# CAS-CLab/quantized-cnn

Measured on AMD Instinct MI355X. Metric: images/sec AlexNet quantized forward, higher is better.
Workload: dtype f32

## Files before the change

### quantized-cnn_amd/csrc/qcnn_decoded.hip

```cpp
#include "qcnn_kernels.h"
#include <algorithm>
#include <type_traits>

typedef float f32x4 __attribute__((ext_vector_type(4)));

#ifndef QCNN_DEC_VAR
#define QCNN_DEC_VAR 0
#endif

namespace {

constexpr int PANEL = QCNN_PANEL;

__device__ __forceinline__ int uni(int v) { return __builtin_amdgcn_readfirstlane(v); }

__host__ __device__ __forceinline__ int qk_dec_krow(int k, int Kr, int Kp) {
  const int last = Kp - 4;
  if (k < last || Kr < 4) return k < Kr ? k : -1;
  const int real = Kr - 4 + (k - last);
  return real >= last ? real : -1;
}

__global__ void k_decode_weights(const uint8_t* __restrict__ rows, const float* __restrict__ ctrd, float* __restrict__ out,
                                 QkSlots sl, int knl, int Cin, int K, int Ct, int Kp, int S) {
  const int total = knl * Kp * S;
  for (int i = blockIdx.x * blockDim.x + threadIdx.x; i < total; i += gridDim.x * blockDim.x) {
    const int ch = i % S, k = qk_dec_krow((i / S) % Kp, knl * Cin, Kp), kh = i / (S * Kp);
    float w = 0.0f;
    if (ch < Ct && k >= 0) {
      const int kw = k / Cin, d = k % Cin;
      const int slot = rows[(size_t)(kh * knl + kw) * sl.rowStride + qk_slot_entry(sl, 0, ch)];
      w = ctrd[(size_t)d * K + qcnn_row_slot(slot)];
    }
    out[i] = w;
  }
}

template <int CT, int PW, bool PADDED, int R, int IT>
__global__ __launch_bounds__(1024) void k_conv_dec(DecParams p) {
  extern __shared__ __attribute__((aligned(16))) float ldsW[];
  const int lane = threadIdx.x & 63, wave = uni(threadIdx.x >> 6);
  const int P = p.Ho * p.Wo;
  {
    const int wq = (p.knl * p.Kp * p.S) >> 2;
    const f32x4* __restrict__ wsrc = reinterpret_cast<const f32x4*>(p.wdec);
    f32x4* ldsW4 = reinterpret_cast<f32x4*>(ldsW);
    for (int i = threadIdx.x; i < wq; i += 1024) ldsW4[i] = wsrc[i];
  }
  __syncthreads();
  const int NS = p.Kp >> 2;
  const int T = p.knl * NS;
  const int groups = (P + PW - 1) / PW;
  constexpr int IB = 16 * IT;
  const int halves = (p.live + IB - 1) / IB;
  const int chunks = p.Ct / (16 * CT);
  const int nItems = p.panels * groups * halves * chunks;
  const int kClamp = p.Kr - 1;
  const int xcd = blockIdx.x & 7, nX = gridDim.x < 8 ? gridDim.x : 8;
  const int wgX = (gridDim.x - xcd + 7) >> 3;
  const int itemBeg = (int)((long long)nItems * xcd / nX), itemEnd = (int)((long long)nItems * (xcd + 1) / nX);
  for (int item = itemBeg + (blockIdx.x >> 3) * 16 + wave; item < itemEnd; item += wgX * 16) {
    int laneI = lane;
    asm volatile("" : "+v"(laneI));
    const int li = laneI & 15, kq = laneI >> 4;
    const int cc = item % chunks, ib = (item / chunks) % halves, pgi = item / (chunks * halves);
    const int panel = pgi / groups, pos0 = (pgi % groups) * PW;
    int r0[PW], c0[PW];
#pragma unroll
    for (int j = 0; j < PW; ++j) {
      const int q = pos0 + j < P ? pos0 + j : P - 1;
      r0[j] = (q / p.Wo) * p.stride - p.pad;
      c0[j] = (q % p.Wo) * p.stride - p.pad;
    }
    const float* __restrict__ srcU = p.src + (size_t)panel * p.H * p.W * p.Cin * PANEL + ib * IB;
    const size_t left = (size_t)(p.panels - panel) * p.H * p.W * p.Cin * PANEL * sizeof(float) - ib * IB * sizeof(float);
    const __amdgpu_buffer_rsrc_t rsrc = __builtin_amdgcn_make_buffer_rsrc(
        const_cast<float*>(srcU), 0, left < 0xffffffffull ? (unsigned)left : 0xffffffffu, 0x00020000);
    const int laneOff = (kq * PANEL + IT * li) * (int)sizeof(float);
    int posOff[PW];
#pragma unroll
    for (int j = 0; j < PW; ++j) posOff[j] = (r0[j] * p.W + c0[j]) * p.Cin * PANEL * (int)sizeof(float);
    const int rowPitch = p.W * p.Cin * PANEL * (int)sizeof(float);
    constexpr int kStep = 4 * PANEL * (int)sizeof(float);
    auto load_b = [&](int kh, int step, int soff, float (&b)[PW][IT]) {
#if QCNN_DEC_VAR & 1
      for (int j = 0; j < PW; ++j) for (int ti = 0; ti < IT; ++ti) b[j][ti] = (float)(kh + step + j + ti);
      return;
#endif
#pragma unroll
      for (int j = 0; j < PW; ++j) {
        if (PADDED) {
          const int row = r0[j] + kh;
          const int k = (step == NS - 1 && p.Kr >= 4) ? p.Kr - 4 + kq : 4 * step + kq;
          const int kc = k < kClamp ? k : kClamp;
          const int col = c0[j] + kc / p.Cin;
          const bool ok = row >= 0 && row < p.H && col >= 0 && col < p.W;
          const float* __restrict__ px = srcU + (ok ? ((row * p.W + c0[j]) * p.Cin + kc) * PANEL + IT * li : 0);
          if (IT == 4) {
            const f32x4 v = *reinterpret_cast<const f32x4*>(px);
#pragma unroll
            for (int ti = 0; ti < IT; ++ti) b[j][ti] = ok ? v[ti] : 0.0f;
          } else {
            const float v = *px;
            b[j][0] = ok ? v : 0.0f;
          }
        } else if (IT == 4) {
          const f32x4 v = __builtin_bit_cast(f32x4, __builtin_amdgcn_raw_buffer_load_b128(rsrc, laneOff, posOff[j] + soff, 0));
#pragma unroll
          for (int ti = 0; ti < IT; ++ti) b[j][ti] = v[ti];
        } else {
          b[j][0] = __builtin_bit_cast(float, __builtin_amdgcn_raw_buffer_load_b32(rsrc, laneOff, posOff[j] + soff, 0));
        }
      }
    };
    f32x4 acc[PW][CT][IT];
#pragma unroll
    for (int ct = 0; ct < CT; ++ct) {
      const f32x4 b4 = *reinterpret_cast<const f32x4*>(p.bias + (cc * CT + ct) * 16 + 4 * kq);
#pragma unroll
      for (int j = 0; j < PW; ++j)
#pragma unroll
        for (int ti = 0; ti < IT; ++ti) acc[j][ct][ti] = b4;
    }
    const int lastOff = NS > 1 ? (p.Kr - 4) * PANEL * (int)sizeof(float) : 0;
    const int incLast = NS > 1 ? lastOff - (NS - 2) * kStep : 0;
    const int incWrap = rowPitch - lastOff;
    int khL = 0, stL = 0, soffL = 0;
    float b[R][PW][IT];
    float a[R][CT];
    auto next_b = [&](float (&bb)[PW][IT]) {
      load_b(khL, stL, soffL, bb);
      const int wrap = stL + 1 == NS ? 1 : 0;
      stL = wrap ? 0 : stL + 1;
      khL += wrap;
      soffL += wrap ? incWrap : (stL == NS - 1 ? incLast : kStep);
    };
    const float* __restrict__ wl = ldsW + kq * p.S + cc * 16 * CT + li;
    const int aStep = 4 * p.S;
    auto load_a = [&](const float* __restrict__ w, float (&aa)[CT]) {
#if QCNN_DEC_VAR & 2
      for (int ct = 0; ct < CT; ++ct) aa[ct] = (float)ct;
      return;
#endif
#pragma unroll
      for (int ct = 0; ct < CT; ++ct) aa[ct] = w[ct * 16];
    };
    auto products = [&](const float (&aa)[CT], const float (&bb)[PW][IT]) {
#pragma unroll
      for (int j = 0; j < PW; ++j)
#pragma unroll
        for (int ti = 0; ti < IT; ++ti)
#pragma unroll
          for (int ct = 0; ct < CT; ++ct)
            acc[j][ct][ti] = __builtin_amdgcn_mfma_f32_16x16x4f32(aa[ct], bb[j][ti], acc[j][ct][ti], 0, 0, 0);
    };
#pragma unroll
    for (int u = 0; u < R; ++u) next_b(b[u]);
    load_a(wl, a[0]);
    int t = 0;
    for (; t + R <= T; t += R) {
#pragma unroll
      for (int u = 0; u < R; ++u) {
        wl += aStep;
        load_a(wl, a[(u + 1) % R]);
        __builtin_amdgcn_sched_barrier(0);
        products(a[u], b[u]);
        __builtin_amdgcn_sched_barrier(0);
        next_b(b[u]);
      }
    }
#pragma unroll
    for (int u = 0; u < R - 1; ++u)
      if (t + u < T) {
        wl += aStep;
        load_a(wl, a[(u + 1) % R]);
        products(a[u], b[u]);
      }
#pragma unroll
    for (int j = 0; j < PW; ++j) {
      if (pos0 + j >= P) continue;
      float* __restrict__ dst = p.dst + ((size_t)panel * P + pos0 + j) * p.Ct * PANEL + ib * IB + IT * li;
#pragma unroll
      for (int ct = 0; ct < CT; ++ct)
#pragma unroll
        for (int r = 0; r < 4; ++r) {
          float v[IT];
#pragma unroll
          for (int ti = 0; ti < IT; ++ti) {
            v[ti] = acc[j][ct][ti][r];
            if (p.relu) v[ti] = (0.0f < v[ti]) ? v[ti] : 0.0f;
          }
          float* __restrict__ o = dst + (size_t)((cc * CT + ct) * 16 + 4 * kq + r) * PANEL;
#if QCNN_DEC_VAR & 8
          if (v[0] == 1.2345f)
#endif
          {
            if (IT == 4) *reinterpret_cast<f32x4*>(o) = f32x4{v[0], v[IT > 1 ? 1 : 0], v[IT > 2 ? 2 : 0], v[IT > 3 ? 3 : 0]};
            else *o = v[0];
          }
        }
    }
  }
}

template <int CT, int PW, bool PADDED, int R, int IT>
hipError_t launch_dec(const DecParams& p, hipStream_t st) {
  const int P = p.Ho * p.Wo;
  const long long items = (long long)p.panels * ((P + PW - 1) / PW) * ((p.live + 16 * IT - 1) / (16 * IT)) * (p.Ct / (16 * CT));
  const int blocks = (int)std::min<long long>(256, (items + 15) / 16);
  const size_t shm = (size_t)p.knl * p.Kp * p.S * sizeof(float);
  auto kern = k_conv_dec<CT, PW, PADDED, R, IT>;
  hipError_t e = hipFuncSetAttribute(reinterpret_cast<const void*>(kern), hipFuncAttributeMaxDynamicSharedMemorySize, (int)shm);
  if (e != hipSuccess) return e;
  hipLaunchKernelGGL(kern, dim3(blocks), dim3(1024), shm, st, p);
  return hipGetLastError();
}

template <int N, int IT>
__device__ __forceinline__ void nchw_wait_impl(float (&bb)[IT]) {
  if constexpr (IT == 4) asm volatile("s_waitcnt vmcnt(%4)" : "+v"(bb[0]), "+v"(bb[1]), "+v"(bb[2]), "+v"(bb[3]) : "n"(N));
  else if constexpr (IT == 5) asm volatile("s_waitcnt vmcnt(%5)" : "+v"(bb[0]), "+v"(bb[1]), "+v"(bb[2]), "+v"(bb[3]), "+v"(bb[4]) : "n"(N));
  else asm volatile("s_waitcnt vmcnt(%6)" : "+v"(bb[0]), "+v"(bb[1]), "+v"(bb[2]), "+v"(bb[3]), "+v"(bb[4]), "+v"(bb[5]) : "n"(N));
}
template <int N, int IT>
__device__ __forceinline__ void nchw_wait(float (&bb)[IT]) { nchw_wait_impl<N, IT>(bb); }

#ifndef NCHW_WAVES
#define NCHW_WAVES 8
#endif
template <int CT, int IT>
__global__ __launch_bounds__(64 * NCHW_WAVES) void k_conv_dec_nchw(DecParams p) {
  static_assert(IT == 4, "a product tile is 2 positions x 8 images, an item two pairs of positions x two image halves");
  extern __shared__ __attribute__((aligned(16))) float ldsW[];
  const int lane = threadIdx.x & 63, wave = uni(threadIdx.x >> 6);
  const int P = p.Ho * p.Wo;
  const int steps = p.Kp >> 2;
  const uint32_t imgBytes = (uint32_t)p.Cin * p.H * p.W * 4u, planeBytes = (uint32_t)p.H * p.W * 4u, rowBytes = (uint32_t)p.W * 4u;
  int* ldsOff = reinterpret_cast<int*>(ldsW + (size_t)(steps + 1) * 4 * p.S);
  {
    const int wq = steps * p.S;
    const f32x4* __restrict__ wsrc = reinterpret_cast<const f32x4*>(p.wdec);
    f32x4* ldsW4 = reinterpret_cast<f32x4*>(ldsW);
    for (int i = threadIdx.x; i < wq; i += 64 * NCHW_WAVES) ldsW4[i] = wsrc[i];
    for (int i = threadIdx.x; i < (steps + 4) * 4; i += 64 * NCHW_WAVES) {
      const int k = min(i, p.Kr - 1);
      const int kw = k % p.knl, kh = (k / p.knl) % p.knl, c = k / (p.knl * p.knl);
      ldsOff[i] = (int)((uint32_t)c * planeBytes + (uint32_t)kh * rowBytes + (uint32_t)kw * 4u);
    }
  }
  __syncthreads();
  const int tiles = (p.live + 15) / 16;
  const int chunks = p.Ct / (16 * CT);
  const int WoG = (p.Wo + IT - 1) / IT, PG = p.Ho * WoG;
  const int nItems = p.panels * PG * tiles * chunks;
  const unsigned long long total = (unsigned long long)p.nImages * imgBytes;
  typedef int i32x4_t __attribute__((ext_vector_type(4)));
  const unsigned long long srcA = reinterpret_cast<unsigned long long>(p.src);
  const i32x4_t rsrc4 = {(int)(unsigned)srcA, (int)((unsigned)(srcA >> 32) & 0xffffu),
                         (int)(total < 0xffffffffull ? (unsigned)total : 0xffffffffu), 0x00020000};
  const int xcd = blockIdx.x & 7, nX = gridDim.x < 8 ? gridDim.x : 8;
  const int wgX = (gridDim.x - xcd + 7) >> 3;
  const int itemBeg = (int)((long long)nItems * xcd / nX), itemEnd = (int)((long long)nItems * (xcd + 1) / nX);
  const bool sparse = itemEnd - itemBeg <= wgX * NCHW_WAVES;
  for (int item = itemBeg + (sparse ? wave * wgX + (int)(blockIdx.x >> 3) : (int)(blockIdx.x >> 3) * NCHW_WAVES + wave); item < itemEnd;
       item += wgX * NCHW_WAVES) {
    int laneI = lane;
    asm volatile("" : "+v"(laneI));
    const int li = laneI & 15, kq = laneI >> 4;
    const int it = item % tiles, cc = (item / tiles) % chunks, pg = (item / (tiles * chunks)) % PG, panel = item / (chunks * tiles * PG);
    const int orow = pg / WoG, ocol = (pg % WoG) * IT;
    const int r0 = orow * p.stride, c0 = ocol * p.stride;
    const uint32_t img0 = (uint32_t)(p.panel0 + panel) * PANEL + (uint32_t)it * 16u;
    const bool edge = img0 + 16u >= (uint32_t)p.nImages;
    const int laneOff = (int)((uint32_t)(li & 7) * imgBytes + (uint32_t)((li >> 3) * p.stride) * 4u);
    const uint32_t base0 = img0 * imgBytes + (uint32_t)(r0 * p.W + c0) * 4u;
    const int* __restrict__ offT = ldsOff + kq;
   auto body = [&](auto edgeTag) {
    constexpr bool EDGE = decltype(edgeTag)::value;
    int laneOffE[IT];
    uint32_t baseE[IT];
    if constexpr (EDGE) {
      const uint32_t lastImg = (uint32_t)p.nImages - 1u, lastPos = (uint32_t)p.Wo - 1u;
#pragma unroll
      for (int ti = 0; ti < IT; ++ti) {
        const uint32_t imgS = min(img0 + 8u * (uint32_t)(ti & 1), lastImg), imgL = min(img0 + 8u * (uint32_t)(ti & 1) + (uint32_t)(li & 7), lastImg);
        const uint32_t posS = min((uint32_t)ocol + 2u * (uint32_t)(ti >> 1), lastPos), posL = min((uint32_t)ocol + 2u * (uint32_t)(ti >> 1) + (uint32_t)(li >> 3), lastPos);
        laneOffE[ti] = (int)((imgL - imgS) * imgBytes + (posL - posS) * (uint32_t)p.stride * 4u);
        baseE[ti] = imgS * imgBytes + ((uint32_t)(r0 * p.W) + posS * (uint32_t)p.stride) * 4u;
      }
    }
#ifndef NCHW_VAR
#define NCHW_VAR 0
#endif
    auto issue = [&, rsrc4, base0](int s, float (&bb)[IT]) {
      const int ot = offT[s * 4];
      const int vo = ot + laneOff;
      (void)base0;
#pragma unroll
      for (int ti = 0; ti < IT; ++ti)
        if (NCHW_VAR & 1) asm volatile("v_mov_b32 %0, %1" : "=v"(bb[ti]) : "v"(vo)); else if constexpr (EDGE)
        asm volatile("buffer_load_dword %0, %1, %2, %3 offen" : "=v"(bb[ti]) : "v"(ot + laneOffE[ti]), "s"(rsrc4), "s"(baseE[ti])); else
        asm volatile("buffer_load_dword %0, %1, %2, %3 offen" : "=v"(bb[ti]) : "v"(vo), "s"(rsrc4),
                     "s"(base0 + (uint32_t)(ti & 1) * 8u * imgBytes + (uint32_t)((ti >> 1) * 2 * p.stride) * 4u));
    };
    f32x4 acc[CT][IT];
#pragma unroll
    for (int ct = 0; ct < CT; ++ct) {
      const float b1 = p.bias[(cc * CT + ct) * 16 + li];
#pragma unroll
      for (int ti = 0; ti < IT; ++ti) acc[ct][ti] = f32x4{b1, b1, b1, b1};
    }
    const float* __restrict__ wl = ldsW + cc * 64 * CT + laneI;
    const int aStep = 4 * p.S;
    float a[2][CT], b[4][IT];
    auto load_a = [&](const float* __restrict__ w, float (&aa)[CT]) {
#pragma unroll
      for (int ct = 0; ct < CT; ++ct) aa[ct] = w[ct * 64];
    };
    issue(0, b[0]);
    issue(1, b[1]);
    issue(2, b[2]);
    load_a(wl, a[0]);
#define NCHW_WAIT(n, bb) nchw_wait<n * IT>(bb)
#define NCHW_STEP(u, n)                                        \
  {                                                                                                                   \
    wl += aStep;                                                                                                      \
    load_a(wl, a[((u) + 1) & 1]);                                                    \
    __builtin_amdgcn_sched_barrier(0);                                                                                \
    NCHW_WAIT(n, b[u]);                                                                                               \
    _Pragma("unroll") for (int ti = 0; ti < IT; ++ti)                                                                 \
      _Pragma("unroll") for (int ct = 0; ct < CT; ++ct)                                                               \
        if (NCHW_VAR & 2) asm volatile("" : "+v"(acc[ct][ti]) : "v"(a[(u) & 1][ct]), "v"(b[u][ti])); else             \
        acc[ct][ti] = __builtin_amdgcn_mfma_f32_16x16x4f32(b[u][ti], a[(u) & 1][ct], acc[ct][ti], 0, 0, 0);           \
    __builtin_amdgcn_sched_barrier(0);                                                                                \
  }
    int s = 0;
    do {
      issue(s + 3, b[3]); NCHW_STEP(0, 3)
      issue(s + 4, b[0]); NCHW_STEP(1, 3)
      issue(s + 5, b[1]); NCHW_STEP(2, 3)
      issue(s + 6, b[2]); NCHW_STEP(3, 3)
    } while ((s += 4) < steps);
    NCHW_WAIT(0, b[0]); NCHW_WAIT(0, b[1]); NCHW_WAIT(0, b[2]);
#undef NCHW_STEP
#undef NCHW_WAIT
    {
      const int nPos = (NCHW_VAR & 4) ? (p.Wo < 0 ? IT : 0) : min(IT, p.Wo - ocol);
      float* __restrict__ dst = p.dst + (((size_t)panel * P + orow * p.Wo + ocol + (kq >> 1)) * p.Ct + li) * PANEL + it * 16 + 4 * (kq & 1);
      if (p.relu) {
#pragma unroll
        for (int tp = 0; tp < IT / 2; ++tp)
          if (tp * 2 + (kq >> 1) < nPos) {
#pragma unroll
            for (int ct = 0; ct < CT; ++ct)
#pragma unroll
              for (int h = 0; h < 2; ++h) {
                const int ti = tp * 2 + h;
                f32x4 v;
#pragma unroll
                for (int e = 0; e < 4; ++e) v[e] = (0.0f < acc[ct][ti][e]) ? acc[ct][ti][e] : 0.0f;
                *reinterpret_cast<f32x4*>(dst + ((size_t)tp * 2 * p.Ct + (cc * CT + ct) * 16) * PANEL + 8 * h) = v;
                __builtin_amdgcn_sched_barrier(0);
              }
          }
      } else {
#pragma unroll
        for (int ti = 0; ti < IT; ++ti)
          if ((ti >> 1) * 2 + (kq >> 1) < nPos) {
#pragma unroll
            for (int ct = 0; ct < CT; ++ct)
              *reinterpret_cast<f32x4*>(dst + ((size_t)(ti >> 1) * 2 * p.Ct + (cc * CT + ct) * 16) * PANEL + 8 * (ti & 1)) = acc[ct][ti];
          }
      }
    }
   };
    if (edge) body(std::true_type{}); else body(std::false_type{});
  }
}

__global__ void k_decode_weights_nchw(const uint8_t* __restrict__ rows, const float* __restrict__ ctrd, float* __restrict__ out,
                                      QkSlots sl, int knl, int Cin, int K, int Ct, int steps, int S) {
  const int total = steps * 4 * S;
  for (int i = blockIdx.x * blockDim.x + threadIdx.x; i < total; i += gridDim.x * blockDim.x) {
    const int ch = (i % 16) + 16 * ((i / 64) % (S / 16)), kq = (i / 16) % 4, step = i / (4 * S);
    const int k = 4 * step + kq;
    float w = 0.0f;
    if (ch < Ct && k < Cin * knl * knl) {
      const int kw = k % knl, kh = (k / knl) % knl, c = k / (knl * knl);
      const int slot = rows[(size_t)(kh * knl + kw) * sl.rowStride + qk_slot_entry(sl, 0, ch)];
      w = ctrd[(size_t)c * K + qcnn_row_slot(slot)];
    }
    out[i] = w;
  }
}

typedef __bf16 bf16x8 __attribute__((ext_vector_type(8)));
typedef __bf16 bf16x2 __attribute__((ext_vector_type(2)));
typedef float f32x2 __attribute__((ext_vector_type(2)));
typedef unsigned u32x4 __attribute__((ext_vector_type(4)));

__device__ __forceinline__ void split_bf16x8(const f32x4 (&x)[2], bf16x8& h1, bf16x8& h2, bf16x8& h3) {
  u32x4 p1, p2, p3;
#pragma unroll
  for (int q = 0; q < 4; ++q) {
    const float x0 = x[q >> 1][2 * (q & 1)], x1 = x[q >> 1][2 * (q & 1) + 1];
    const unsigned a = __builtin_bit_cast(unsigned, __builtin_convertvector(f32x2{x0, x1}, bf16x2));
    const float r0 = x0 - __builtin_bit_cast(float, a << 16), r1 = x1 - __builtin_bit_cast(float, a & 0xffff0000u);
    const unsigned b = __builtin_bit_cast(unsigned, __builtin_convertvector(f32x2{r0, r1}, bf16x2));
    const float s0 = r0 - __builtin_bit_cast(float, b << 16), s1 = r1 - __builtin_bit_cast(float, b & 0xffff0000u);
    p1[q] = a; p2[q] = b;
    p3[q] = __builtin_bit_cast(unsigned, __builtin_convertvector(f32x2{s0, s1}, bf16x2));
  }
  h1 = __builtin_bit_cast(bf16x8, p1); h2 = __builtin_bit_cast(bf16x8, p2); h3 = __builtin_bit_cast(bf16x8, p3);
}

template <int N>
__device__ __forceinline__ void split_wait(f32x4 (&x)[4][2]) {
  asm volatile("s_waitcnt vmcnt(%8)" : "+v"(x[0][0]), "+v"(x[0][1]), "+v"(x[1][0]), "+v"(x[1][1]), "+v"(x[2][0]), "+v"(x[2][1]),
               "+v"(x[3][0]), "+v"(x[3][1]) : "n"(N));
}
template <int N>
__device__ __forceinline__ void split_wait(u32x4& w) { asm volatile("s_waitcnt vmcnt(%1)" : "+v"(w) : "n"(N)); }

template <int CT, int IT>
__global__ __launch_bounds__(64 * NCHW_WAVES) void k_conv_dec_nchw_split(DecParams p) {
  static_assert(IT == 4 && CT == 6, "a product tile is 2 positions x 8 images, an item two pairs of positions x two image halves x 96 channels");
  extern __shared__ __attribute__((aligned(16))) float ldsW[];
  const int lane = threadIdx.x & 63, wave = uni(threadIdx.x >> 6);
  const int P = p.Ho * p.Wo;
  const int steps = p.Kp >> 5;
  const int CTs = p.S >> 4;
  const uint32_t imgBytes = (uint32_t)p.Cin * p.H * p.W * 4u, planeBytes = (uint32_t)p.H * p.W * 4u, rowBytes = (uint32_t)p.W * 4u;
  int* ldsOff = reinterpret_cast<int*>(ldsW + (size_t)p.Kp * p.S);
  {
    const int wq = (p.Kp * p.S) >> 2;
    const f32x4* __restrict__ wsrc = reinterpret_cast<const f32x4*>(p.wdec);
    f32x4* ldsW4 = reinterpret_cast<f32x4*>(ldsW);
    for (int i = threadIdx.x; i < wq; i += 64 * NCHW_WAVES) ldsW4[i] = wsrc[i];
    for (int i = threadIdx.x; i < p.Kp + 32; i += 64 * NCHW_WAVES) {
      const int k = min(i, p.Kr - 1);
      const int kw = k % p.knl, kh = (k / p.knl) % p.knl, c = k / (p.knl * p.knl);
      ldsOff[i] = (int)((uint32_t)c * planeBytes + (uint32_t)kh * rowBytes + (uint32_t)kw * 4u);
    }
  }
  __syncthreads();
  const int tiles = (p.live + 15) / 16;
  const int chunks = p.Ct / (16 * CT);
  const int WoG = (p.Wo + IT - 1) / IT, PG = p.Ho * WoG;
  const int nItems = p.panels * PG * tiles * chunks;
  const unsigned long long total = (unsigned long long)p.nImages * imgBytes;
  typedef int i32x4_t __attribute__((ext_vector_type(4)));
  const unsigned long long srcA = reinterpret_cast<unsigned long long>(p.src);
  const i32x4_t rsrc4 = {(int)(unsigned)srcA, (int)((unsigned)(srcA >> 32) & 0xffffu),
                         (int)(total < 0xffffffffull ? (unsigned)total : 0xffffffffu), 0x00020000};
  const unsigned long long w3A = reinterpret_cast<unsigned long long>(p.wdec) + (size_t)p.Kp * p.S * 4;
  const uint32_t w3Bytes = (uint32_t)p.Kp * p.S * 2u, w3Step = (uint32_t)p.S * 64u;
  const i32x4_t rsrcW = {(int)(unsigned)w3A, (int)((unsigned)(w3A >> 32) & 0xffffu), (int)w3Bytes, 0x00020000};
  const int xcd = blockIdx.x & 7, nX = gridDim.x < 8 ? gridDim.x : 8;
  const int wgX = (gridDim.x - xcd + 7) >> 3;
  const int itemBeg = (int)((long long)nItems * xcd / nX), itemEnd = (int)((long long)nItems * (xcd + 1) / nX);
  const bool sparse = itemEnd - itemBeg <= wgX * NCHW_WAVES;
  for (int item = itemBeg + (sparse ? wave * wgX + (int)(blockIdx.x >> 3) : (int)(blockIdx.x >> 3) * NCHW_WAVES + wave); item < itemEnd;
       item += wgX * NCHW_WAVES) {
    int laneI = lane;
    asm volatile("" : "+v"(laneI));
    const int li = laneI & 15, kg = laneI >> 4;
    const int it = item % tiles, cc = (item / tiles) % chunks, pg = (item / (tiles * chunks)) % PG, panel = item / (chunks * tiles * PG);
    const int orow = pg / WoG, ocol = (pg % WoG) * IT;
    const int r0 = orow * p.stride, c0 = ocol * p.stride;
    const uint32_t img0 = (uint32_t)(p.panel0 + panel) * PANEL + (uint32_t)it * 16u;
    const bool edge = img0 + 16u >= (uint32_t)p.nImages;
    const int laneOff = (int)((uint32_t)(li & 7) * imgBytes + (uint32_t)((li >> 3) * p.stride) * 4u);
    const uint32_t base0 = img0 * imgBytes + (uint32_t)(r0 * p.W + c0) * 4u;
   auto body = [&](auto edgeTag) {
    constexpr bool EDGE = decltype(edgeTag)::value;
    int laneOffE[IT];
    uint32_t baseS[IT];
#pragma unroll
    for (int ti = 0; ti < IT; ++ti) {
      laneOffE[ti] = laneOff;
      baseS[ti] = base0 + (uint32_t)(ti & 1) * 8u * imgBytes + (uint32_t)((ti >> 1) * 2 * p.stride) * 4u;
    }
    if constexpr (EDGE) {
      const uint32_t lastImg = (uint32_t)p.nImages - 1u, lastPos = (uint32_t)p.Wo - 1u;
#pragma unroll
      for (int ti = 0; ti < IT; ++ti) {
        const uint32_t imgS = min(img0 + 8u * (uint32_t)(ti & 1), lastImg), imgL = min(img0 + 8u * (uint32_t)(ti & 1) + (uint32_t)(li & 7), lastImg);
        const uint32_t posS = min((uint32_t)ocol + 2u * (uint32_t)(ti >> 1), lastPos), posL = min((uint32_t)ocol + 2u * (uint32_t)(ti >> 1) + (uint32_t)(li >> 3), lastPos);
        laneOffE[ti] = (int)((imgL - imgS) * imgBytes + (posL - posS) * (uint32_t)p.stride * 4u);
        baseS[ti] = imgS * imgBytes + ((uint32_t)(r0 * p.W) + posS * (uint32_t)p.stride) * 4u;
      }
    }
    const int* __restrict__ offT = ldsOff + 8 * kg;
    f32x4 xr[IT][2];
    auto issue_x = [&, rsrc4](int s) {
      const i32x4_t o0 = *reinterpret_cast<const i32x4_t*>(offT + 32 * s), o1 = *reinterpret_cast<const i32x4_t*>(offT + 32 * s + 4);
      const int ot[8] = {o0[0], o0[1], o0[2], o0[3], o1[0], o1[1], o1[2], o1[3]};
#pragma unroll
      for (int ti = 0; ti < IT; ++ti)
#pragma unroll
        for (int j = 0; j < 8; ++j) {
          float v;
          if (NCHW_VAR & 1) asm volatile("v_mov_b32 %0, %1" : "=v"(v) : "v"(ot[j]));
          else asm volatile("buffer_load_dword %0, %1, %2, %3 offen" : "=v"(v) : "v"(ot[j] + laneOffE[ti]), "s"(rsrc4), "s"(baseS[ti]));
          xr[ti][j >> 2][j & 3] = v;
        }
    };
    u32x4 w3[CT];
    const int w3Lane = lane * 16;
    auto issue_w3 = [&, rsrcW, w3Step](int s, int ct) {
      if (NCHW_VAR & 16) asm volatile("v_mov_b32 %0, %1" : "=v"(w3[ct][0]) : "v"(s)); else
      asm volatile("buffer_load_dwordx4 %0, %1, %2, %3 offen" : "=v"(w3[ct]) : "v"(w3Lane + (int)(s * w3Step)), "s"(rsrcW),
                   "s"((uint32_t)((cc * CT + ct) * 1024)));
    };
    f32x4 acc[CT][IT];
#pragma unroll
    for (int ct = 0; ct < CT; ++ct) {
      const float b1 = p.bias[(cc * CT + ct) * 16 + li];
#pragma unroll
      for (int ti = 0; ti < IT; ++ti) acc[ct][ti] = f32x4{b1, b1, b1, b1};
    }
    const u32x4* __restrict__ wl = reinterpret_cast<const u32x4*>(ldsW) + (size_t)(cc * CT) * 128 + lane;
    const int wStep = CTs * 128;
    issue_x(0);
#pragma unroll
    for (int ct = 0; ct < CT; ++ct) issue_w3(0, ct);
    int s = 0;
    do {
      u32x4 bw[2][2];
      bw[0][0] = wl[0]; bw[0][1] = wl[64];
      split_wait<CT>(xr);
      bf16x8 a1[IT], a2[IT], a3[IT];
#pragma unroll
      for (int ti = 0; ti < IT; ++ti) {
        if (NCHW_VAR & 8) {
          a1[ti] = __builtin_bit_cast(bf16x8, xr[ti][0]);
          a2[ti] = a1[ti]; a3[ti] = a1[ti];
        } else {
          split_bf16x8(xr[ti], a1[ti], a2[ti], a3[ti]);
        }
      }
      __builtin_amdgcn_sched_barrier(0);
      issue_x(s + 1);
      __builtin_amdgcn_sched_barrier(0);
#pragma unroll
      for (int ct = 0; ct < CT; ++ct) {
        if (ct + 1 < CT) { bw[(ct + 1) & 1][0] = wl[(ct + 1) * 128]; bw[(ct + 1) & 1][1] = wl[(ct + 1) * 128 + 64]; }
        split_wait<CT - 1 + 8 * IT>(w3[ct]);
        const bf16x8 b1 = __builtin_bit_cast(bf16x8, bw[ct & 1][0]), b2 = __builtin_bit_cast(bf16x8, bw[ct & 1][1]);
        const bf16x8 b3 = __builtin_bit_cast(bf16x8, w3[ct]);
#define SPLIT_TERM(A, B)                                                                                               \
  _Pragma("unroll") for (int ti = 0; ti < IT; ++ti)                                                                    \
    if (NCHW_VAR & 2) asm volatile("" : "+v"(acc[ct][ti]) : "v"(A[ti]), "v"(B)); else                                  \
    acc[ct][ti] = __builtin_amdgcn_mfma_f32_16x16x32_bf16(A[ti], B, acc[ct][ti], 0, 0, 0);
        SPLIT_TERM(a3, b1) SPLIT_TERM(a2, b2) SPLIT_TERM(a1, b3) SPLIT_TERM(a2, b1) SPLIT_TERM(a1, b2) SPLIT_TERM(a1, b1)
#undef SPLIT_TERM
        __builtin_amdgcn_sched_barrier(0);
        issue_w3(s + 1, ct);
        __builtin_amdgcn_sched_barrier(0);
      }
      wl += wStep;
    } while (++s < steps);
    split_wait<0>(xr);
#pragma unroll
    for (int ct = 0; ct < CT; ++ct) split_wait<0>(w3[ct]);
    {
      const int nPos = (NCHW_VAR & 4) ? (p.Wo < 0 ? IT : 0) : min(IT, p.Wo - ocol);
      float* __restrict__ dst = p.dst + (((size_t)panel * P + orow * p.Wo + ocol + (kg >> 1)) * p.Ct + li) * PANEL + it * 16 + 4 * (kg & 1);
      if (p.relu) {
#pragma unroll
        for (int tp = 0; tp < IT / 2; ++tp)
          if (tp * 2 + (kg >> 1) < nPos) {
#pragma unroll
            for (int ct = 0; ct < CT; ++ct)
#pragma unroll
              for (int h = 0; h < 2; ++h) {
                const int ti = tp * 2 + h;
                f32x4 v;
#pragma unroll
                for (int e = 0; e < 4; ++e) v[e] = (0.0f < acc[ct][ti][e]) ? acc[ct][ti][e] : 0.0f;
                *reinterpret_cast<f32x4*>(dst + ((size_t)tp * 2 * p.Ct + (cc * CT + ct) * 16) * PANEL + 8 * h) = v;
                __builtin_amdgcn_sched_barrier(0);
              }
          }
      } else {
#pragma unroll
        for (int ti = 0; ti < IT; ++ti)
          if ((ti >> 1) * 2 + (kg >> 1) < nPos) {
#pragma unroll
            for (int ct = 0; ct < CT; ++ct)
              *reinterpret_cast<f32x4*>(dst + ((size_t)(ti >> 1) * 2 * p.Ct + (cc * CT + ct) * 16) * PANEL + 8 * (ti & 1)) = acc[ct][ti];
          }
      }
    }
   };
    if (edge) body(std::true_type{}); else body(std::false_type{});
  }
}

__device__ __forceinline__ float bf16_hi(float x, uint16_t* h) {
  uint32_t u = __builtin_bit_cast(uint32_t, x);
  u += 0x7fffu + ((u >> 16) & 1u);
  *h = (uint16_t)(u >> 16);
  return __builtin_bit_cast(float, u & 0xffff0000u);
}

__global__ void k_decode_weights_split(const uint8_t* __restrict__ rows, const float* __restrict__ ctrd, uint16_t* __restrict__ out,
                                       QkSlots sl, int knl, int Cin, int K, int Ct, int Kb, int S) {
  const int total = Kb * S, CTs = S / 16;
  uint16_t* __restrict__ out3 = out + (size_t)2 * total;
  for (int i = blockIdx.x * blockDim.x + threadIdx.x; i < total; i += gridDim.x * blockDim.x) {
    const int j = i & 7, ln = (i >> 3) & 63, tile = (i >> 9) % CTs, step = (i >> 9) / CTs;
    const int ch = 16 * tile + (ln & 15), k = 32 * step + 8 * (ln >> 4) + j;
    float w = 0.0f;
    if (ch < Ct && k < Cin * knl * knl) {
      const int kw = k % knl, kh = (k / knl) % knl, c = k / (knl * knl);
      const int slot = rows[(size_t)(kh * knl + kw) * sl.rowStride + qk_slot_entry(sl, 0, ch)];
      w = ctrd[(size_t)c * K + qcnn_row_slot(slot)];
    }
    uint16_t h1, h2, h3;
    const float r = w - bf16_hi(w, &h1);
    (void)bf16_hi(r - bf16_hi(r, &h2), &h3);
    const size_t blk = (size_t)(step * CTs + tile) * 2 * 512 + ln * 8 + j;
    out[blk] = h1;
    out[blk + 512] = h2;
    out3[i] = h3;
  }
}

__global__ __launch_bounds__(1024) void k_fc_dec(FcDecParams p) {
  extern __shared__ __attribute__((aligned(16))) float ldsR[];
  const int lane = threadIdx.x & 63, wave = uni(threadIdx.x >> 6);
  const int li = lane & 15, kq = lane >> 4;
  const int cb = blockIdx.x, half = blockIdx.y % p.halves, panel = blockIdx.y / p.halves, z = blockIdx.z;
  const int steps = p.D / (4 * 16 * (int)gridDim.z);
  const int k0 = (z * 16 + wave) * steps * 4;
  const __amdgpu_buffer_rsrc_t ra = __builtin_amdgcn_make_buffer_rsrc(
      const_cast<float*>(p.wdec), 0, (unsigned)((size_t)p.D * p.S * sizeof(float)), 0x00020000);
  const float* __restrict__ xb = p.src + (size_t)panel * p.D * PANEL;
  const __amdgpu_buffer_rsrc_t rb = __builtin_amdgcn_make_buffer_rsrc(
      const_cast<float*>(xb), 0, (unsigned)((size_t)p.D * PANEL * sizeof(float)), 0x00020000);
  const int aLane = (kq * p.S + cb * 64 + 4 * li) * (int)sizeof(float);
  const int bLane = (kq * PANEL + half * 64 + 4 * li) * (int)sizeof(float);
  const int aStep = 4 * p.S * (int)sizeof(float), bStep = 4 * PANEL * (int)sizeof(float);
  f32x4 acc[4][4];
#pragma unroll
  for (int ct = 0; ct < 4; ++ct)
#pragma unroll
    for (int ti = 0; ti < 4; ++ti) acc[ct][ti] = f32x4{0.0f, 0.0f, 0.0f, 0.0f};
  constexpr int R = 3;
  f32x4 a[R], b[R];
  int aoff = k0 * p.S * (int)sizeof(float), boff = k0 * PANEL * (int)sizeof(float);
  auto next = [&](f32x4& aa, f32x4& bb) {
    aa = __builtin_bit_cast(f32x4, __builtin_amdgcn_raw_buffer_load_b128(ra, aLane, aoff, 0));
    bb = __builtin_bit_cast(f32x4, __builtin_amdgcn_raw_buffer_load_b128(rb, bLane, boff, 0));
    aoff += aStep; boff += bStep;
  };
  auto products = [&](const f32x4& aa, const f32x4& bb) {
#pragma unroll
    for (int ct = 0; ct < 4; ++ct)
#pragma unroll
      for (int ti = 0; ti < 4; ++ti) acc[ct][ti] = __builtin_amdgcn_mfma_f32_16x16x4f32(aa[ct], bb[ti], acc[ct][ti], 0, 0, 0);
  };
#pragma unroll
  for (int u = 0; u < R; ++u) next(a[u], b[u]);
  int t = 0;
  for (; t + R <= steps; t += R) {
#pragma unroll
    for (int u = 0; u < R; ++u) {
      products(a[u], b[u]);
      __builtin_amdgcn_sched_barrier(0);
      next(a[u], b[u]);
    }
  }
#pragma unroll
  for (int u = 0; u < R - 1; ++u)
    if (t + u < steps) products(a[u], b[u]);
  f32x4* lds4 = reinterpret_cast<f32x4*>(ldsR);
#pragma unroll
  for (int stride = 8; stride >= 1; stride >>= 1) {
    if (wave >= stride && wave < 2 * stride) {
#pragma unroll
      for (int i = 0; i < 16; ++i) lds4[((wave - stride) * 16 + i) * 64 + lane] = acc[i >> 2][i & 3];
    }
    __syncthreads();
    if (wave < stride) {
#pragma unroll
      for (int i = 0; i < 16; ++i) {
        const f32x4 v = lds4[(wave * 16 + i) * 64 + lane];
        acc[i >> 2][i & 3] += v;
      }
    }
    __syncthreads();
  }
  if (wave != 0) return;
  float* __restrict__ out = (gridDim.z > 1 ? p.partial + (size_t)z * p.panels * p.Ct * PANEL : p.dst) +
                            (size_t)panel * p.Ct * PANEL + half * 64 + 4 * li;
  const bool first = z == 0;
#pragma unroll
  for (int ct = 0; ct < 4; ++ct)
#pragma unroll
    for (int r = 0; r < 4; ++r) {
      const int ch = cb * 64 + 4 * (4 * kq + r) + ct;
      if (ch < p.Ct) {
        const float bv = first ? p.bias[ch] : 0.0f;
        f32x4 v = {acc[ct][0][r] + bv, acc[ct][1][r] + bv, acc[ct][2][r] + bv, acc[ct][3][r] + bv};
        if (p.relu && gridDim.z == 1) {
          v[0] = (0.0f < v[0]) ? v[0] : 0.0f; v[1] = (0.0f < v[1]) ? v[1] : 0.0f;
          v[2] = (0.0f < v[2]) ? v[2] : 0.0f; v[3] = (0.0f < v[3]) ? v[3] : 0.0f;
        }
        *reinterpret_cast<f32x4*>(out + (size_t)ch * PANEL) = v;
      }
    }
}

__global__ void k_decode_fc_weights(const uint8_t* __restrict__ rows, const float* __restrict__ ctrd, float* __restrict__ out,
                                    QkSlots sl, int D, int K, int Ct, int S) {
  const int G = qcnn_stage_group(K);
  const size_t total = (size_t)D * S;
  for (size_t i = blockIdx.x * (size_t)blockDim.x + threadIdx.x; i < total; i += (size_t)gridDim.x * blockDim.x) {
    const int ch = (int)(i % S), k = (int)(i / S);
    float w = 0.0f;
    if (ch < Ct) {
      const int slot = rows[(size_t)k * sl.rowStride + qk_slot_entry(sl, 0, ch)];
      w = ctrd[(size_t)k * K + (qcnn_row_slot(slot) - (k % G) * K)];
    }
    out[i] = w;
  }
}

}

bool qk_conv_dec_shape(int Cin, int grp, int M, int Ct, int knl, int* Kp, int* S) {
  if (grp != 1 || M != 1 || Cin < 1 || Cin > 4) return false;
  if (Ct < 32 || Ct % 32) return false;
  const int kp = (knl * Cin + 3) / 4 * 4;
  const size_t lim = 160 * 1024;
  int s = Ct;
  while ((s & 63) != 16 && (s & 63) != 48) s += 16;
  if ((size_t)knl * kp * s * sizeof(float) > lim) s = Ct;
  if ((size_t)knl * kp * s * sizeof(float) > lim) return false;
  *Kp = kp; *S = s;
  return true;
}

hipError_t qk_decode_weights(const uint8_t* rows, const float* ctrd, float* out, const QkSlots& sl, int knl, int Cin, int K,
                             int Ct, int Kp, int S, hipStream_t st) {
  const int total = knl * Kp * S;
  hipLaunchKernelGGL(k_decode_weights, dim3((total + 255) / 256), dim3(256), 0, st, rows, ctrd, out, sl, knl, Cin, K, Ct, Kp, S);
  return hipGetLastError();
}

hipError_t qk_conv_dec(const DecParams& p, hipStream_t st) {
  if ((long long)p.H * p.W * p.Cin * QCNN_PANEL * 4 >= (1ll << 31)) return hipErrorInvalidValue;
  if (p.Ct % 32) return hipErrorInvalidValue;
  const bool clamped = p.pad || p.Kr < 4;
  if (p.live <= 16) {
    if (clamped) return launch_dec<2, 4, true, 2, 1>(p, st);
    if (p.Ct % 96 == 0) return launch_dec<6, 2, false, 3, 1>(p, st);
    if (p.Ct % 64 == 0) return launch_dec<4, 4, false, 3, 1>(p, st);
    return launch_dec<2, 6, false, 3, 1>(p, st);
  }
  if (clamped) {
    if (p.Ct % 64 == 0) return launch_dec<4, 1, true, 2, 4>(p, st);
    return launch_dec<2, 1, true, 3, 4>(p, st);
  }
  if (p.Ct % 96 == 0) {
    const long long items = (long long)p.panels * p.Ho * p.Wo * ((p.live + 63) / 64) * (p.Ct / 96);
    if (items > 4096 && items < 2 * 4096) return launch_dec<3, 1, false, 3, 4>(p, st);
    return launch_dec<6, 1, false, 2, 4>(p, st);
  }
  if (p.Ct % 64 == 0) return launch_dec<4, 1, false, 3, 4>(p, st);
  return launch_dec<2, 2, false, 3, 4>(p, st);
}

bool qk_fc_dec_shape(int D, int M, int Cs, int Ct, int* S) {
  if (Cs != 1 || M != D || D % 64 || Ct < 1) return false;
  if ((size_t)D * PANEL * sizeof(float) >= (1ull << 32)) return false;
  *S = (Ct + 63) / 64 * 64;
  return (size_t)D * *S * sizeof(float) < (1ull << 32);
}

hipError_t qk_decode_fc_weights(const uint8_t* rows, const float* ctrd, float* out, const QkSlots& sl, int D, int K, int Ct,
                                int S, hipStream_t st) {
  hipLaunchKernelGGL(k_decode_fc_weights, dim3(2048), dim3(256), 0, st, rows, ctrd, out, sl, D, K, Ct, S);
  return hipGetLastError();
}

int qk_fc_dec_slices(int D, int Ct, int panels, int live) {
  const int wgs = ((Ct + 63) / 64) * panels * ((live + 63) / 64);
  int z = 1;
  while (wgs * z < 192 && D % (64 * 2 * z) == 0 && D / (64 * 2 * z) >= 4 && 2 * z <= 32) z *= 2;
  return z;
}

hipError_t qk_fc_dec(const FcDecParams& p, int slices, int live, hipStream_t st) {
  if (p.D % (64 * slices)) return hipErrorInvalidValue;
  FcDecParams q = p;
  q.halves = (live + 63) / 64;
  const dim3 grid((unsigned)((p.Ct + 63) / 64), (unsigned)(p.panels * q.halves), (unsigned)slices);
  const size_t shm = 8 * 16 * 256 * sizeof(float);
  hipError_t e = hipFuncSetAttribute(reinterpret_cast<const void*>(k_fc_dec), hipFuncAttributeMaxDynamicSharedMemorySize, (int)shm);
  if (e != hipSuccess) return e;
  hipLaunchKernelGGL(k_fc_dec, grid, dim3(1024), shm, st, q);
  return hipGetLastError();
}

bool qk_conv_dec_nchw_shape(int Cin, int grp, int M, int Ct, int knl, int pad, int* Kp, int* S) {
  if (grp != 1 || M != 1 || Cin < 1 || Cin > 4 || pad != 0 || Ct % 96) return false;
  const int kp = (Cin * knl * knl + 15) / 16 * 16;
  if ((size_t)(kp + 4) * Ct * sizeof(float) + (kp / 4 + 4) * 16 > 160 * 1024) return false;
  *Kp = kp; *S = Ct;
  return true;
}

hipError_t qk_decode_weights_nchw(const uint8_t* rows, const float* ctrd, float* out, const QkSlots& sl, int knl, int Cin, int K,
                                  int Ct, int Kp, int S, hipStream_t st) {
  const int total = Kp * S;
  hipLaunchKernelGGL(k_decode_weights_nchw, dim3((total + 255) / 256), dim3(256), 0, st, rows, ctrd, out, sl, knl, Cin, K, Ct, Kp / 4, S);
  return hipGetLastError();
}

hipError_t qk_conv_dec_nchw(const DecParams& p, hipStream_t st) {
  if (!p.srcNchw || p.pad != 0 || p.Ct % 96 || p.S != p.Ct || (unsigned long long)p.nImages * p.Cin * p.H * p.W * 4ull >= (1ull << 32))
    return hipErrorInvalidValue;
  const long long items = (long long)p.panels * p.Ho * ((p.Wo + 3) / 4) * ((p.live + 15) / 16) * (p.Ct / 96);
  const int blocks = (int)std::min<long long>(256, items);
  const size_t shm = (size_t)(p.Kp + 4) * p.S * sizeof(float) + (size_t)(p.Kp / 4 + 4) * 16;
  auto kern = k_conv_dec_nchw<6, 4>;
  hipError_t e = hipFuncSetAttribute(reinterpret_cast<const void*>(kern), hipFuncAttributeMaxDynamicSharedMemorySize, (int)shm);
  if (e != hipSuccess) return e;
  hipLaunchKernelGGL(kern, dim3(blocks), dim3(64 * NCHW_WAVES), shm, st, p);
  return hipGetLastError();
}

bool qk_conv_dec_nchw_split_shape(int Cin, int grp, int M, int Ct, int knl, int pad, int* Kb) {
  int kp = 0, s = 0;
  if (!qk_conv_dec_nchw_shape(Cin, grp, M, Ct, knl, pad, &kp, &s)) return false;
  const int kb = (Cin * knl * knl + 31) / 32 * 32;
  if ((size_t)kb * Ct * 4 + (size_t)(kb + 32) * 4 > 160 * 1024) return false;
  *Kb = kb;
  return true;
}

hipError_t qk_decode_weights_split(const uint8_t* rows, const float* ctrd, uint16_t* out, const QkSlots& sl, int knl, int Cin, int K,
                                   int Ct, int Kb, hipStream_t st) {
  const int total = Kb * Ct;
  hipLaunchKernelGGL(k_decode_weights_split, dim3((total + 255) / 256), dim3(256), 0, st, rows, ctrd, out, sl, knl, Cin, K, Ct, Kb, Ct);
  return hipGetLastError();
}

hipError_t qk_conv_dec_nchw_split(const DecParams& p, hipStream_t st) {
  if (!p.srcNchw || p.pad != 0 || p.Ct % 96 || p.S != p.Ct || p.Kp % 32 || (unsigned long long)p.nImages * p.Cin * p.H * p.W * 4ull >= (1ull << 32))
    return hipErrorInvalidValue;
  const long long items = (long long)p.panels * p.Ho * ((p.Wo + 3) / 4) * ((p.live + 15) / 16) * (p.Ct / 96);
  const int blocks = (int)std::min<long long>(256, items);
  const size_t shm = (size_t)p.Kp * p.S * 4 + (size_t)(p.Kp + 32) * 4;
  auto kern = k_conv_dec_nchw_split<6, 4>;
  hipError_t e = hipFuncSetAttribute(reinterpret_cast<const void*>(kern), hipFuncAttributeMaxDynamicSharedMemorySize, (int)shm);
  if (e != hipSuccess) return e;
  hipLaunchKernelGGL(kern, dim3(blocks), dim3(64 * NCHW_WAVES), shm, st, p);
  return hipGetLastError();
}
```

Measured before the change: 105,000.

## Reorder split conv K dimension into 4-wide kernel-row runs for dwordx4 input loads

Adds a RUNS variant of the split NCHW decoded conv that lays out the reduction dimension as runs of 4 consecutive kw taps per (c,kh). With that layout each lane fetches its 8 input values with two buffer_load_dwordx4 instead of eight scalar dword loads. The offset table shrinks to one entry per run. The weight decoder pads each run, duplicating overlap at the row end and zeroing the overlapped taps. This adds padding work to K (e.g. 11 taps become 12 for AlexNet conv1) and relies on 16-byte loads into unaligned addresses.

```diff
diff --git a/quantized-cnn_amd/csrc/qcnn_decoded.hip b/quantized-cnn_amd/csrc/qcnn_decoded.hip
--- a/quantized-cnn_amd/csrc/qcnn_decoded.hip
+++ b/quantized-cnn_amd/csrc/qcnn_decoded.hip
@@ -422,7 +422,17 @@
 template <int N>
 __device__ __forceinline__ void split_wait(u32x4& w) { asm volatile("s_waitcnt vmcnt(%1)" : "+v"(w) : "n"(N)); }
 
-template <int CT, int IT>
+static inline int nchw_split_kb(int Cin, int knl, int nr) { return nr ? (Cin * knl * nr + 7) / 8 * 32 : (Cin * knl * knl + 31) / 32 * 32; }
+static inline size_t nchw_split_lds(int Kb, int Ct, int nr) {
+  return (size_t)Kb * Ct * 4 + (size_t)(nr ? Kb / 4 + 8 : Kb + 32) * 4;
+}
+static int nchw_split_runs(int Cin, int knl, int Ct) {
+  if (knl < 4) return 0;
+  const int nr = (knl + 3) / 4;
+  return nchw_split_lds(nchw_split_kb(Cin, knl, nr), Ct, nr) <= 160 * 1024 ? nr : 0;
+}
+
+template <int CT, int IT, bool RUNS>
 __global__ __launch_bounds__(64 * NCHW_WAVES) void k_conv_dec_nchw_split(DecParams p) {
   static_assert(IT == 4 && CT == 6, "a product tile is 2 positions x 8 images, an item two pairs of positions x two image halves x 96 channels");
   extern __shared__ __attribute__((aligned(16))) float ldsW[];
@@ -437,10 +447,19 @@
     const f32x4* __restrict__ wsrc = reinterpret_cast<const f32x4*>(p.wdec);
     f32x4* ldsW4 = reinterpret_cast<f32x4*>(ldsW);
     for (int i = threadIdx.x; i < wq; i += 64 * NCHW_WAVES) ldsW4[i] = wsrc[i];
-    for (int i = threadIdx.x; i < p.Kp + 32; i += 64 * NCHW_WAVES) {
-      const int k = min(i, p.Kr - 1);
-      const int kw = k % p.knl, kh = (k / p.knl) % p.knl, c = k / (p.knl * p.knl);
-      ldsOff[i] = (int)((uint32_t)c * planeBytes + (uint32_t)kh * rowBytes + (uint32_t)kw * 4u);
+    if constexpr (RUNS) {
+      const int nr = (p.knl + 3) >> 2, nRuns = p.Cin * p.knl * nr;
+      for (int i = threadIdx.x; i < (p.Kp >> 2) + 8; i += 64 * NCHW_WAVES) {
+        const int r = min(i, nRuns - 1);
+        const int kw = min(4 * (r % nr), p.knl - 4), kh = (r / nr) % p.knl, c = r / (nr * p.knl);
+        ldsOff[i] = (int)((uint32_t)c * planeBytes + (uint32_t)kh * rowBytes + (uint32_t)kw * 4u);
+      }
+    } else {
+      for (int i = threadIdx.x; i < p.Kp + 32; i += 64 * NCHW_WAVES) {
+        const int k = min(i, p.Kr - 1);
+        const int kw = k % p.knl, kh = (k / p.knl) % p.knl, c = k / (p.knl * p.knl);
+        ldsOff[i] = (int)((uint32_t)c * planeBytes + (uint32_t)kh * rowBytes + (uint32_t)kw * 4u);
+      }
     }
   }
   __syncthreads();
@@ -491,9 +510,25 @@
         baseS[ti] = imgS * imgBytes + ((uint32_t)(r0 * p.W) + posS * (uint32_t)p.stride) * 4u;
       }
     }
-    const int* __restrict__ offT = ldsOff + 8 * kg;
+    const int* __restrict__ offT = ldsOff + (RUNS ? 2 : 8) * kg;
     f32x4 xr[IT][2];
     auto issue_x = [&, rsrc4](int s) {
+      if constexpr (RUNS) {
+        typedef int i32x2_t __attribute__((ext_vector_type(2)));
+        const i32x2_t o = *reinterpret_cast<const i32x2_t*>(offT + 8 * s);
+#pragma unroll
+        for (int ti = 0; ti < IT; ++ti)
+#pragma unroll
+          for (int h = 0; h < 2; ++h) {
+            if (NCHW_VAR & 1) {
+              float v;
+              asm volatile("v_mov_b32 %0, %1" : "=v"(v) : "v"(o[h]));
+              xr[ti][h] = f32x4{v, v, v, v};
+            } else
+            asm volatile("buffer_load_dwordx4 %0, %1, %2, %3 offen" : "=v"(xr[ti][h]) : "v"(o[h] + laneOffE[ti]), "s"(rsrc4), "s"(baseS[ti]));
+          }
+        return;
+      }
       const i32x4_t o0 = *reinterpret_cast<const i32x4_t*>(offT + 32 * s), o1 = *reinterpret_cast<const i32x4_t*>(offT + 32 * s + 4);
       const int ot[8] = {o0[0], o0[1], o0[2], o0[3], o1[0], o1[1], o1[2], o1[3]};
 #pragma unroll
@@ -525,6 +560,7 @@
     issue_x(0);
 #pragma unroll
     for (int ct = 0; ct < CT; ++ct) issue_w3(0, ct);
+    constexpr int xLoads = (RUNS ? 2 : 8) * IT;
     int s = 0;
     do {
       u32x4 bw[2][2];
@@ -546,7 +582,7 @@
 #pragma unroll
       for (int ct = 0; ct < CT; ++ct) {
         if (ct + 1 < CT) { bw[(ct + 1) & 1][0] = wl[(ct + 1) * 128]; bw[(ct + 1) & 1][1] = wl[(ct + 1) * 128 + 64]; }
-        split_wait<CT - 1 + 8 * IT>(w3[ct]);
+        split_wait<CT - 1 + xLoads>(w3[ct]);
         const bf16x8 b1 = __builtin_bit_cast(bf16x8, bw[ct & 1][0]), b2 = __builtin_bit_cast(bf16x8, bw[ct & 1][1]);
         const bf16x8 b3 = __builtin_bit_cast(bf16x8, w3[ct]);
 #define SPLIT_TERM(A, B)                                                                                               \
@@ -606,15 +642,21 @@
 }
 
 __global__ void k_decode_weights_split(const uint8_t* __restrict__ rows, const float* __restrict__ ctrd, uint16_t* __restrict__ out,
-                                       QkSlots sl, int knl, int Cin, int K, int Ct, int Kb, int S) {
+                                       QkSlots sl, int knl, int Cin, int K, int Ct, int Kb, int S, int nr) {
   const int total = Kb * S, CTs = S / 16;
   uint16_t* __restrict__ out3 = out + (size_t)2 * total;
   for (int i = blockIdx.x * blockDim.x + threadIdx.x; i < total; i += gridDim.x * blockDim.x) {
     const int j = i & 7, ln = (i >> 3) & 63, tile = (i >> 9) % CTs, step = (i >> 9) / CTs;
     const int ch = 16 * tile + (ln & 15), k = 32 * step + 8 * (ln >> 4) + j;
     float w = 0.0f;
-    if (ch < Ct && k < Cin * knl * knl) {
-      const int kw = k % knl, kh = (k / knl) % knl, c = k / (knl * knl);
+    int kw = k % knl, kh = (k / knl) % knl, c = k / (knl * knl);
+    bool live = k < Cin * knl * knl;
+    if (nr) {
+      const int r = k >> 2, ri = r % nr;
+      kw = min(4 * ri, knl - 4) + (k & 3); kh = (r / nr) % knl; c = r / (nr * knl);
+      live = r < Cin * knl * nr && kw >= 4 * ri;
+    }
+    if (ch < Ct && live) {
       const int slot = rows[(size_t)(kh * knl + kw) * sl.rowStride + qk_slot_entry(sl, 0, ch)];
       w = ctrd[(size_t)c * K + qcnn_row_slot(slot)];
     }
@@ -837,8 +879,9 @@
 bool qk_conv_dec_nchw_split_shape(int Cin, int grp, int M, int Ct, int knl, int pad, int* Kb) {
   int kp = 0, s = 0;
   if (!qk_conv_dec_nchw_shape(Cin, grp, M, Ct, knl, pad, &kp, &s)) return false;
-  const int kb = (Cin * knl * knl + 31) / 32 * 32;
-  if ((size_t)kb * Ct * 4 + (size_t)(kb + 32) * 4 > 160 * 1024) return false;
+  const int nr = nchw_split_runs(Cin, knl, Ct);
+  const int kb = nchw_split_kb(Cin, knl, nr);
+  if (nchw_split_lds(kb, Ct, nr) > 160 * 1024) return false;
   *Kb = kb;
   return true;
 }
@@ -846,17 +889,21 @@
 hipError_t qk_decode_weights_split(const uint8_t* rows, const float* ctrd, uint16_t* out, const QkSlots& sl, int knl, int Cin, int K,
                                    int Ct, int Kb, hipStream_t st) {
   const int total = Kb * Ct;
-  hipLaunchKernelGGL(k_decode_weights_split, dim3((total + 255) / 256), dim3(256), 0, st, rows, ctrd, out, sl, knl, Cin, K, Ct, Kb, Ct);
+  const int nr = nchw_split_runs(Cin, knl, Ct);
+  if (Kb != nchw_split_kb(Cin, knl, nr)) return hipErrorInvalidValue;
+  hipLaunchKernelGGL(k_decode_weights_split, dim3((total + 255) / 256), dim3(256), 0, st, rows, ctrd, out, sl, knl, Cin, K, Ct, Kb, Ct, nr);
   return hipGetLastError();
 }
 
 hipError_t qk_conv_dec_nchw_split(const DecParams& p, hipStream_t st) {
-  if (!p.srcNchw || p.pad != 0 || p.Ct % 96 || p.S != p.Ct || p.Kp % 32 || (unsigned long long)p.nImages * p.Cin * p.H * p.W * 4ull >= (1ull << 32))
+  const int nr = nchw_split_runs(p.Cin, p.knl, p.Ct);
+  if (!p.srcNchw || p.pad != 0 || p.Ct % 96 || p.S != p.Ct || p.Kp != nchw_split_kb(p.Cin, p.knl, nr) ||
+      (unsigned long long)p.nImages * p.Cin * p.H * p.W * 4ull >= (1ull << 32))
     return hipErrorInvalidValue;
   const long long items = (long long)p.panels * p.Ho * ((p.Wo + 3) / 4) * ((p.live + 15) / 16) * (p.Ct / 96);
   const int blocks = (int)std::min<long long>(256, items);
-  const size_t shm = (size_t)p.Kp * p.S * 4 + (size_t)(p.Kp + 32) * 4;
-  auto kern = k_conv_dec_nchw_split<6, 4>;
+  const size_t shm = nchw_split_lds(p.Kp, p.S, nr);
+  auto kern = nr ? k_conv_dec_nchw_split<6, 4, true> : k_conv_dec_nchw_split<6, 4, false>;
   hipError_t e = hipFuncSetAttribute(reinterpret_cast<const void*>(kern), hipFuncAttributeMaxDynamicSharedMemorySize, (int)shm);
   if (e != hipSuccess) return e;
   hipLaunchKernelGGL(kern, dim3(blocks), dim3(64 * NCHW_WAVES), shm, st, p);
```

Result: faster. 107,000, median of 6 (+1.9%).
